# qirui-chen/RGA3-release

Measured on AMD Instinct MI355X. Metric: video-QA samples/sec (fwd+bwd) at 7B/16-frame — full RGA3 training step (Qwen2.5-VL-7B + SAM2-L + mask losses + AdamW), higher is better.
Workload: dtype bf16

## Files before the change

rga3-release_amd/csrc/attn_args.h:

```cpp
#pragma once
#include "common.h"

namespace rga3 {

struct AttnArgs {
    const unsigned short* q;
    const unsigned short* k;
    const unsigned short* v;
    unsigned short* o;
    float* lse;
    const int* cu_q;
    const int* cu_k;
    long q_st, q_sh, k_st, k_sh, v_st, v_sh, o_st, o_sh;
    int Hq, Hkv, D;
    long total_q;
    float scale_log2;
    int causal;
    float* split_o;
    float* split_lse;
    int nsplit;
    int bq_shift, bk_shift;
    const float* rope_cos;
    const float* rope_sin;
    const float* rope_kcos;
    const float* rope_ksin;
    int gx;
};

int launch_causal32(const AttnArgs& a, int nseg, int max_q, hipStream_t st);

}
```

rga3-release_amd/csrc/attn_bwd.hip:

```cpp
#include "common.h"

#include <mutex>
#include <set>

namespace rga3 {

struct AttnBwdArgs {
    const unsigned short *q, *k, *v, *o, *dout;
    unsigned short *dq, *dk, *dv;
    const float* lse;
    float* delta;
    const int *cu_q, *cu_k;
    long q_st, q_sh, k_st, k_sh, v_st, v_sh, o_st, o_sh, do_st, do_sh, dq_st, dq_sh, dk_st, dk_sh, dv_st, dv_sh;
    int Hq, Hkv, D;
    long total_q;
    float scale, scale_log2;
    int causal;
    float* dkv_ws;
    long total_k;
    int gx, gy;
};

constexpr int BT = 64;

template <int DP, int QT, int NWAVE, bool PAIR>
__global__ __launch_bounds__(64 * NWAVE) void attn_bwd_dq_kernel(AttnBwdArgs p) {
    constexpr int NT = 64 * NWAVE;
    constexpr int BLOCK_M = NWAVE * QT * 16;
    constexpr int CH = DP / 8;
    constexpr int STRIDE = DP * 2 + 32;
    constexpr int DS = DP / 32, DT = DP / 16;
    constexpr int LOADS = (BT * CH) / NT;
    static_assert((BT * CH) % NT == 0, "tile chunks must divide evenly over threads");

    extern __shared__ __attribute__((aligned(16))) char smem[];
    char* Ks = smem;
    char* Vs = smem + BT * STRIDE;

    const int tid = threadIdx.x, lane = tid & 63;
    const int wid = __builtin_amdgcn_readfirstlane(tid >> 6);
    const int g = lane >> 4, c = lane & 15;
    const Wg3 wg = xcd_decode3(p.gx, p.gy);
    const int seg = wg.z, hq = wg.y;
    const int hk = hq / (p.Hq / p.Hkv);
    const int qs = p.cu_q[seg], Lq = p.cu_q[seg + 1] - qs;
    const int ks = p.cu_k[seg], Lk = p.cu_k[seg + 1] - ks;
    const int shift = Lk - Lq;
    const int nqb = (Lq + BLOCK_M - 1) / BLOCK_M;
    int qb_first = wg.x, qb_second = -1;
    if constexpr (PAIR) {
        qb_first = nqb - 1 - wg.x;
        qb_second = wg.x;
        if (qb_second > qb_first) return;
        if (qb_second == qb_first) qb_second = -1;
    } else if (qb_first >= nqb) {
        return;
    }
    for (int pass = 0; pass < (PAIR ? 2 : 1); ++pass) {
    const int qbi = pass == 0 ? qb_first : qb_second;
    if (qbi < 0) break;
    if (pass == 1) __syncthreads();
    const int qb0 = qbi * BLOCK_M;
    const int qw0 = qb0 + wid * (QT * 16);

    bf16x8 qf[QT][DS], dof[QT][DS];
    float lse2[QT], dl[QT];
#pragma unroll
    for (int t = 0; t < QT; ++t) {
        const int qi = qw0 + t * 16 + c;
        const bool ok = qi < Lq;
#pragma unroll
        for (int ds = 0; ds < DS; ++ds) {
            const int d = ds * 32 + g * 8;
            u32x4 z = {0u, 0u, 0u, 0u}, y = {0u, 0u, 0u, 0u};
            if (ok && d < p.D) {
                z = *(const u32x4*)(p.q + (long)(qs + qi) * p.q_st + (long)hq * p.q_sh + d);
                y = *(const u32x4*)(p.dout + (long)(qs + qi) * p.do_st + (long)hq * p.do_sh + d);
            }
            qf[t][ds] = __builtin_bit_cast(bf16x8, z);
            dof[t][ds] = __builtin_bit_cast(bf16x8, y);
        }
        lse2[t] = ok ? p.lse[(long)hq * p.total_q + qs + qi] * 1.4426950408889634f : 0.f;
    }
#pragma unroll
    for (int t = 0; t < QT; ++t) {
        const int qi = qw0 + t * 16 + c;
        const bool ok = qi < Lq;
        float dp = 0.f;
#pragma unroll
        for (int ds = 0; ds < DS; ++ds) {
            const int d = ds * 32 + g * 8;
            if (ok && d < p.D) {
                const u32x4 ov = *(const u32x4*)(p.o + (long)(qs + qi) * p.o_st + (long)hq * p.o_sh + d);
                const u32x4 dv = __builtin_bit_cast(u32x4, dof[t][ds]);
#pragma unroll
                for (int i = 0; i < 4; ++i) {
                    dp += __uint_as_float(ov[i] << 16) * __uint_as_float(dv[i] << 16);
                    dp += __uint_as_float(ov[i] & 0xffff0000u) * __uint_as_float(dv[i] & 0xffff0000u);
                }
            }
        }
        dp += __shfl_xor(dp, 16, 64);
        dp += __shfl_xor(dp, 32, 64);
        dl[t] = ok ? dp : 0.f;
        if (ok && g == 0) p.delta[(long)hq * p.total_q + qs + qi] = dp;
    }

    f32x4 dqacc[QT][DT];
#pragma unroll
    for (int t = 0; t < QT; ++t)
#pragma unroll
        for (int d = 0; d < DT; ++d) dqacc[t][d] = f32x4{0.f, 0.f, 0.f, 0.f};

    int kv_end = Lk;
    if (p.causal) kv_end = min(Lk, qb0 + BLOCK_M + shift);
    if (kv_end < 0) kv_end = 0;
    const int ntiles = (kv_end + BT - 1) / BT;

    u32x4 kreg[LOADS], vreg[LOADS];
    auto load_tile = [&](int kt) {
#pragma unroll
        for (int i = 0; i < LOADS; ++i) {
            const int idx = tid + i * NT;
            const int r = idx / CH, ch = idx % CH;
            const int key = kt * BT + r;
            u32x4 zk = {0u, 0u, 0u, 0u}, zv = {0u, 0u, 0u, 0u};
            if (key < Lk && ch * 8 < p.D) {
                zk = *(const u32x4*)(p.k + (long)(ks + key) * p.k_st + (long)hk * p.k_sh + ch * 8);
                zv = *(const u32x4*)(p.v + (long)(ks + key) * p.v_st + (long)hk * p.v_sh + ch * 8);
            }
            kreg[i] = zk;
            vreg[i] = zv;
        }
    };
    auto store_tile = [&]() {
#pragma unroll
        for (int i = 0; i < LOADS; ++i) {
            const int idx = tid + i * NT;
            const int r = idx / CH, ch = idx % CH;
            *(u32x4*)(Ks + r * STRIDE + ch * 16) = kreg[i];
            *(u32x4*)(Vs + r * STRIDE + ch * 16) = vreg[i];
        }
    };

    if (ntiles > 0) load_tile(0);
    for (int kt = 0; kt < ntiles; ++kt) {
        __syncthreads();
        store_tile();
        __syncthreads();
        if (kt + 1 < ntiles) load_tile(kt + 1);
        const int k0 = kt * BT;
        const bool need_mask = (k0 + BT > Lk) || (p.causal && (k0 + BT - 1 > qb0 + shift));
#pragma unroll
        for (int t = 0; t < QT; ++t) {
            const int qi = qw0 + t * 16 + c;
            f32x4 s[4], dp[4];
#pragma unroll
            for (int j = 0; j < 4; ++j) { s[j] = f32x4{0.f, 0.f, 0.f, 0.f}; dp[j] = f32x4{0.f, 0.f, 0.f, 0.f}; }
#pragma unroll
            for (int j = 0; j < 4; ++j)
#pragma unroll
                for (int ds = 0; ds < DS; ++ds) {
                    bf16x8 kf = *(const bf16x8*)(Ks + (j * 16 + c) * STRIDE + ds * 64 + g * 16);
                    bf16x8 vf = *(const bf16x8*)(Vs + (j * 16 + c) * STRIDE + ds * 64 + g * 16);
                    s[j] = __builtin_amdgcn_mfma_f32_16x16x32_bf16(kf, qf[t][ds], s[j], 0, 0, 0);
                    dp[j] = __builtin_amdgcn_mfma_f32_16x16x32_bf16(vf, dof[t][ds], dp[j], 0, 0, 0);
                }
            bf16x8 dsf[2];
#pragma unroll
            for (int ss = 0; ss < 2; ++ss) {
                float e[8];
#pragma unroll
                for (int u = 0; u < 8; ++u) {
                    const int j = 2 * ss + (u >> 2), r = u & 3;
                    float pr = __builtin_amdgcn_exp2f(s[j][r] * p.scale_log2 - lse2[t]);
                    if (need_mask) {
                        const int key = k0 + j * 16 + 4 * g + r;
                        const bool ok = (key < Lk) && (!p.causal || key <= qi + shift);
                        pr = ok ? pr : 0.f;
                    }
                    if (qi >= Lq) pr = 0.f;
                    e[u] = pr * (dp[j][r] - dl[t]) * p.scale;
                }
                u32x4 pk;
                pk[0] = pack_bf2(e[0], e[1]); pk[1] = pack_bf2(e[2], e[3]); pk[2] = pack_bf2(e[4], e[5]); pk[3] = pack_bf2(e[6], e[7]);
                dsf[ss] = __builtin_bit_cast(bf16x8, pk);
            }
#pragma unroll
            for (int d = 0; d < DT; ++d)
#pragma unroll
                for (int ss = 0; ss < 2; ++ss) {
                    const char* a0 = Ks + (ss * 32 + 4 * g + (c >> 2)) * STRIDE + (d * 16 + 4 * (c & 3)) * 2;
                    bf16x4 lo = __builtin_amdgcn_ds_read_tr16_b64_v4bf16((__attribute__((address_space(3))) bf16x4*)(a0));
                    bf16x4 hi = __builtin_amdgcn_ds_read_tr16_b64_v4bf16((__attribute__((address_space(3))) bf16x4*)(a0 + 16 * STRIDE));
                    bf16x8 kt8;
                    kt8[0] = lo[0]; kt8[1] = lo[1]; kt8[2] = lo[2]; kt8[3] = lo[3];
                    kt8[4] = hi[0]; kt8[5] = hi[1]; kt8[6] = hi[2]; kt8[7] = hi[3];
                    dqacc[t][d] = __builtin_amdgcn_mfma_f32_16x16x32_bf16(kt8, dsf[ss], dqacc[t][d], 0, 0, 0);
                }
        }
    }
#pragma unroll
    for (int t = 0; t < QT; ++t) {
        const int qi = qw0 + t * 16 + c;
        if (qi < Lq) {
            unsigned short* row = p.dq + (long)(qs + qi) * p.dq_st + (long)hq * p.dq_sh;
#pragma unroll
            for (int d = 0; d < DT; ++d) {
                const int dd = d * 16 + 4 * g;
                if (dd < p.D) {
                    u32x2 pk;
                    pk[0] = pack_bf2(dqacc[t][d][0], dqacc[t][d][1]);
                    pk[1] = pack_bf2(dqacc[t][d][2], dqacc[t][d][3]);
                    *(u32x2*)(row + dd) = pk;
                }
            }
        }
    }
    }
}

template <int DP, int NWAVE, bool SPLIT, bool PAIR>
__global__ __launch_bounds__(64 * NWAVE) void attn_bwd_dkv_kernel(AttnBwdArgs p) {
    constexpr int NT = 64 * NWAVE;
    constexpr int BLOCK_N = NWAVE * 16;
    constexpr int CH = DP / 8;
    constexpr int STRIDE = DP * 2 + 32;
    constexpr int DS = DP / 32, DT = DP / 16;
    constexpr int LOADS = (BT * CH) / NT;
    static_assert((BT * CH) % NT == 0, "tile chunks must divide evenly over threads");

    extern __shared__ __attribute__((aligned(16))) char smem[];
    char* Qs = smem;
    char* Os = smem + BT * STRIDE;
    float* Ls = (float*)(smem + 2 * BT * STRIDE);

    const int tid = threadIdx.x, lane = tid & 63;
    const int wid = __builtin_amdgcn_readfirstlane(tid >> 6);
    const int g = lane >> 4, c = lane & 15;
    const Wg3 wg = xcd_decode3(p.gx, p.gy);
    const int seg = wg.z;
    const int group = p.Hq / p.Hkv;
    const int hk = SPLIT ? wg.y / group : wg.y;
    const int hh0 = SPLIT ? wg.y % group : 0, hh1 = SPLIT ? hh0 + 1 : group;
    const int qs = p.cu_q[seg], Lq = p.cu_q[seg + 1] - qs;
    const int ks = p.cu_k[seg], Lk = p.cu_k[seg + 1] - ks;
    const int shift = Lk - Lq;
    const int nkb = (Lk + BLOCK_N - 1) / BLOCK_N;
    int kb_first = wg.x, kb_second = -1;
    if constexpr (PAIR) {
        kb_first = wg.x;
        kb_second = nkb - 1 - wg.x;
        if (kb_first > kb_second) return;
        if (kb_second == kb_first) kb_second = -1;
    } else if (kb_first >= nkb) {
        return;
    }
    for (int pass = 0; pass < (PAIR ? 2 : 1); ++pass) {
    const int kbi = pass == 0 ? kb_first : kb_second;
    if (kbi < 0) break;
    if (pass == 1) __syncthreads();
    const int kb0 = kbi * BLOCK_N;
    const int key = kb0 + wid * 16 + c;

    bf16x8 kf[DS], vf[DS];
#pragma unroll
    for (int ds = 0; ds < DS; ++ds) {
        const int d = ds * 32 + g * 8;
        u32x4 z = {0u, 0u, 0u, 0u}, y = {0u, 0u, 0u, 0u};
        if (key < Lk && d < p.D) {
            z = *(const u32x4*)(p.k + (long)(ks + key) * p.k_st + (long)hk * p.k_sh + d);
            y = *(const u32x4*)(p.v + (long)(ks + key) * p.v_st + (long)hk * p.v_sh + d);
        }
        kf[ds] = __builtin_bit_cast(bf16x8, z);
        vf[ds] = __builtin_bit_cast(bf16x8, y);
    }
    f32x4 dkacc[DT], dvacc[DT];
#pragma unroll
    for (int d = 0; d < DT; ++d) { dkacc[d] = f32x4{0.f, 0.f, 0.f, 0.f}; dvacc[d] = f32x4{0.f, 0.f, 0.f, 0.f}; }

    int q_begin = 0;
    if (p.causal) q_begin = max(0, kb0 - shift);
    const int t0 = q_begin / BT;
    const int ntq = (Lq + BT - 1) / BT;

    u32x4 qreg[LOADS], oreg[LOADS];
    float lreg = 0.f, dreg = 0.f;
    auto load_tile = [&](int hq_, int qt_) {
#pragma unroll
        for (int i = 0; i < LOADS; ++i) {
            const int idx = tid + i * NT;
            const int r = idx / CH, ch = idx % CH;
            const int qi = qt_ * BT + r;
            u32x4 zq = {0u, 0u, 0u, 0u}, zo = {0u, 0u, 0u, 0u};
            if (qi < Lq && ch * 8 < p.D) {
                zq = *(const u32x4*)(p.q + (long)(qs + qi) * p.q_st + (long)hq_ * p.q_sh + ch * 8);
                zo = *(const u32x4*)(p.dout + (long)(qs + qi) * p.do_st + (long)hq_ * p.do_sh + ch * 8);
            }
            qreg[i] = zq;
            oreg[i] = zo;
        }
        if (tid < BT) {
            const int qi = qt_ * BT + tid;
            lreg = (qi < Lq) ? p.lse[(long)hq_ * p.total_q + qs + qi] * 1.4426950408889634f : 0.f;
            dreg = (qi < Lq) ? p.delta[(long)hq_ * p.total_q + qs + qi] : 0.f;
        }
    };
    auto store_tile = [&]() {
#pragma unroll
        for (int i = 0; i < LOADS; ++i) {
            const int idx = tid + i * NT;
            const int r = idx / CH, ch = idx % CH;
            *(u32x4*)(Qs + r * STRIDE + ch * 16) = qreg[i];
            *(u32x4*)(Os + r * STRIDE + ch * 16) = oreg[i];
        }
        if (tid < BT) {
            Ls[tid] = lreg;
            Ls[BT + tid] = dreg;
        }
    };
    if (t0 < ntq) load_tile(hk * group + hh0, t0);
    for (int hh = hh0; hh < hh1; ++hh) {
        const int hq = hk * group + hh;
        for (int qt = t0; qt < ntq; ++qt) {
            __syncthreads();
            store_tile();
            __syncthreads();
            if (qt + 1 < ntq) load_tile(hq, qt + 1);
            else if (hh + 1 < hh1) load_tile(hq + 1, t0);
            const int q0 = qt * BT;
            f32x4 s[4], dp[4];
#pragma unroll
            for (int j = 0; j < 4; ++j) { s[j] = f32x4{0.f, 0.f, 0.f, 0.f}; dp[j] = f32x4{0.f, 0.f, 0.f, 0.f}; }
#pragma unroll
            for (int j = 0; j < 4; ++j)
#pragma unroll
                for (int ds = 0; ds < DS; ++ds) {
                    bf16x8 qa = *(const bf16x8*)(Qs + (j * 16 + c) * STRIDE + ds * 64 + g * 16);
                    bf16x8 oa = *(const bf16x8*)(Os + (j * 16 + c) * STRIDE + ds * 64 + g * 16);
                    s[j] = __builtin_amdgcn_mfma_f32_16x16x32_bf16(qa, kf[ds], s[j], 0, 0, 0);
                    dp[j] = __builtin_amdgcn_mfma_f32_16x16x32_bf16(oa, vf[ds], dp[j], 0, 0, 0);
                }
            bf16x8 pf[2], dsf[2];
#pragma unroll
            for (int ss = 0; ss < 2; ++ss) {
                float e[8], f[8];
#pragma unroll
                for (int u = 0; u < 8; ++u) {
                    const int j = 2 * ss + (u >> 2), r = u & 3;
                    const int ql = j * 16 + 4 * g + r;
                    const int qi = q0 + ql;
                    float pr = __builtin_amdgcn_exp2f(s[j][r] * p.scale_log2 - Ls[ql]);
                    const bool ok = (qi < Lq) && (key < Lk) && (!p.causal || key <= qi + shift);
                    pr = ok ? pr : 0.f;
                    e[u] = pr;
                    f[u] = pr * (dp[j][r] - Ls[BT + ql]) * p.scale;
                }
                u32x4 a, b;
                a[0] = pack_bf2(e[0], e[1]); a[1] = pack_bf2(e[2], e[3]); a[2] = pack_bf2(e[4], e[5]); a[3] = pack_bf2(e[6], e[7]);
                b[0] = pack_bf2(f[0], f[1]); b[1] = pack_bf2(f[2], f[3]); b[2] = pack_bf2(f[4], f[5]); b[3] = pack_bf2(f[6], f[7]);
                pf[ss] = __builtin_bit_cast(bf16x8, a);
                dsf[ss] = __builtin_bit_cast(bf16x8, b);
            }
#pragma unroll
            for (int d = 0; d < DT; ++d)
#pragma unroll
                for (int ss = 0; ss < 2; ++ss) {
                    const int roff = (ss * 32 + 4 * g + (c >> 2)) * STRIDE + (d * 16 + 4 * (c & 3)) * 2;
                    bf16x4 ol = __builtin_amdgcn_ds_read_tr16_b64_v4bf16((__attribute__((address_space(3))) bf16x4*)(Os + roff));
                    bf16x4 oh = __builtin_amdgcn_ds_read_tr16_b64_v4bf16((__attribute__((address_space(3))) bf16x4*)(Os + roff + 16 * STRIDE));
                    bf16x4 ql_ = __builtin_amdgcn_ds_read_tr16_b64_v4bf16((__attribute__((address_space(3))) bf16x4*)(Qs + roff));
                    bf16x4 qh_ = __builtin_amdgcn_ds_read_tr16_b64_v4bf16((__attribute__((address_space(3))) bf16x4*)(Qs + roff + 16 * STRIDE));
                    bf16x8 ot, qt8;
                    ot[0] = ol[0]; ot[1] = ol[1]; ot[2] = ol[2]; ot[3] = ol[3]; ot[4] = oh[0]; ot[5] = oh[1]; ot[6] = oh[2]; ot[7] = oh[3];
                    qt8[0] = ql_[0]; qt8[1] = ql_[1]; qt8[2] = ql_[2]; qt8[3] = ql_[3]; qt8[4] = qh_[0]; qt8[5] = qh_[1]; qt8[6] = qh_[2]; qt8[7] = qh_[3];
                    dvacc[d] = __builtin_amdgcn_mfma_f32_16x16x32_bf16(ot, pf[ss], dvacc[d], 0, 0, 0);
                    dkacc[d] = __builtin_amdgcn_mfma_f32_16x16x32_bf16(qt8, dsf[ss], dkacc[d], 0, 0, 0);
                }
        }
    }
    if constexpr (SPLIT) {
        if (key < Lk) {
            const long half = (long)group * p.total_k * p.Hkv * p.D;
            float* wk = p.dkv_ws + (((long)hh0 * p.total_k + ks + key) * p.Hkv + hk) * p.D;
#pragma unroll
            for (int d = 0; d < DT; ++d) {
                const int dd = d * 16 + 4 * g;
                if (dd < p.D) {
                    *(f32x4*)(wk + dd) = dkacc[d];
                    *(f32x4*)(wk + half + dd) = dvacc[d];
                }
            }
        }
        continue;
    }
    if (key < Lk) {
        unsigned short* rk = p.dk + (long)(ks + key) * p.dk_st + (long)hk * p.dk_sh;
        unsigned short* rv = p.dv + (long)(ks + key) * p.dv_st + (long)hk * p.dv_sh;
#pragma unroll
        for (int d = 0; d < DT; ++d) {
            const int dd = d * 16 + 4 * g;
            if (dd < p.D) {
                u32x2 a, b;
                a[0] = pack_bf2(dkacc[d][0], dkacc[d][1]); a[1] = pack_bf2(dkacc[d][2], dkacc[d][3]);
                b[0] = pack_bf2(dvacc[d][0], dvacc[d][1]); b[1] = pack_bf2(dvacc[d][2], dvacc[d][3]);
                *(u32x2*)(rk + dd) = a;
                *(u32x2*)(rv + dd) = b;
            }
        }
    }
    }
}

__global__ __launch_bounds__(256) void attn_dkv_reduce_kernel(AttnBwdArgs p) {
    const int group = p.Hq / p.Hkv;
    const int d4 = p.D / 4;
    const long idx = (long)blockIdx.x * 256 + threadIdx.x;
    const long total = p.total_k * p.Hkv * d4;
    if (idx >= total) return;
    const int dd = (int)(idx % d4) * 4;
    const long row = idx / d4;
    const int hk = (int)(row % p.Hkv);
    const long key = row / p.Hkv;
    const long plane = p.total_k * p.Hkv * (long)p.D, half = (long)group * plane;
    const float* w = p.dkv_ws + row * p.D + dd;
    f32x4 sk = *(const f32x4*)w, sv = *(const f32x4*)(w + half);
    for (int h = 1; h < group; ++h) {
        sk += *(const f32x4*)(w + h * plane);
        sv += *(const f32x4*)(w + half + h * plane);
    }
    u32x2 a, b;
    a[0] = pack_bf2(sk[0], sk[1]); a[1] = pack_bf2(sk[2], sk[3]);
    b[0] = pack_bf2(sv[0], sv[1]); b[1] = pack_bf2(sv[2], sv[3]);
    *(u32x2*)(p.dk + key * p.dk_st + (long)hk * p.dk_sh + dd) = a;
    *(u32x2*)(p.dv + key * p.dv_st + (long)hk * p.dv_sh + dd) = b;
}

template <int DP>
static int launch_bwd(const AttnBwdArgs& a0, int nseg, int max_q, int max_k, hipStream_t st) {
    AttnBwdArgs a = a0;
    a.gx = 1; a.gy = 1;
    constexpr int NW = (DP == 128) ? 8 : 4;
#ifdef RGA3_BWD_DQ_QT2
    constexpr int QT = 2, NWQ = 4;
#else
    constexpr int QT = (DP >= 128) ? 1 : 2, NWQ = NW;
#endif
    constexpr int BLOCK_M = NWQ * QT * 16;
    constexpr int LDS_DQ = 2 * BT * (DP * 2 + 32);
    constexpr int LDS_DKV = 2 * BT * (DP * 2 + 32) + 2 * BT * 4;
    auto prep = [](const void* k, int lds) -> int {
        if (lds <= 48 * 1024) return 0;
        static std::mutex mu;
        static std::set<std::pair<const void*, int>> done;
        int dev = 0;
        if (hipGetDevice(&dev) != hipSuccess) dev = 0;
        std::lock_guard<std::mutex> lk(mu);
        if (done.count({k, dev})) return 0;
        hipError_t e = hipFuncSetAttribute(k, hipFuncAttributeMaxDynamicSharedMemorySize, lds);
        if (e != hipSuccess) return fail(-(int)e, "attn_bwd: hipFuncSetAttribute: %s", hipGetErrorString(e));
        done.insert({k, dev});
        return 0;
    };
    const unsigned nqb = (unsigned)cdiv(max_q, BLOCK_M), nkb = (unsigned)cdiv(max_k, 16 * NW);
    const bool pair = a.causal && nqb >= 4 && nkb >= 4;
    if (pair) {
        auto kq = attn_bwd_dq_kernel<DP, QT, NWQ, true>;
        if (int rc = prep((const void*)kq, LDS_DQ)) return rc;
        a.gx = (int)((nqb + 1) / 2); a.gy = a.Hq;
        hipLaunchKernelGGL(kq, dim3((unsigned)a.gx * (unsigned)a.gy * (unsigned)nseg), dim3(64 * NWQ), LDS_DQ, st, a);
    } else {
        auto kq = attn_bwd_dq_kernel<DP, QT, NWQ, false>;
        if (int rc = prep((const void*)kq, LDS_DQ)) return rc;
        a.gx = (int)nqb; a.gy = a.Hq;
        hipLaunchKernelGGL(kq, dim3((unsigned)a.gx * (unsigned)a.gy * (unsigned)nseg), dim3(64 * NWQ), LDS_DQ, st, a);
    }
    RGA3_CHECK_LAUNCH("attn_bwd_dq_kernel");
    const unsigned gx = pair ? (nkb + 1) / 2 : nkb;
    if (a.dkv_ws && a.Hq > a.Hkv) {
        if (pair) {
            auto ks_ = attn_bwd_dkv_kernel<DP, NW, true, true>;
            if (int rc = prep((const void*)ks_, LDS_DKV)) return rc;
            a.gx = (int)gx; a.gy = a.Hq;
            hipLaunchKernelGGL(ks_, dim3((unsigned)a.gx * (unsigned)a.gy * (unsigned)nseg), dim3(64 * NW), LDS_DKV, st, a);
        } else {
            auto ks_ = attn_bwd_dkv_kernel<DP, NW, true, false>;
            if (int rc = prep((const void*)ks_, LDS_DKV)) return rc;
            a.gx = (int)gx; a.gy = a.Hq;
            hipLaunchKernelGGL(ks_, dim3((unsigned)a.gx * (unsigned)a.gy * (unsigned)nseg), dim3(64 * NW), LDS_DKV, st, a);
        }
        RGA3_CHECK_LAUNCH("attn_bwd_dkv_kernel<split>");
        const long rows = a.total_k * a.Hkv;
        hipLaunchKernelGGL(attn_dkv_reduce_kernel, dim3((unsigned)cdiv(rows * (a.D / 4), 256)), dim3(256), 0, st, a);
        RGA3_CHECK_LAUNCH("attn_dkv_reduce_kernel");
        return 0;
    }
    if (pair) {
        auto kk = attn_bwd_dkv_kernel<DP, NW, false, true>;
        if (int rc = prep((const void*)kk, LDS_DKV)) return rc;
        a.gx = (int)gx; a.gy = a.Hkv;
        hipLaunchKernelGGL(kk, dim3((unsigned)a.gx * (unsigned)a.gy * (unsigned)nseg), dim3(64 * NW), LDS_DKV, st, a);
    } else {
        auto kk = attn_bwd_dkv_kernel<DP, NW, false, false>;
        if (int rc = prep((const void*)kk, LDS_DKV)) return rc;
        a.gx = (int)gx; a.gy = a.Hkv;
        hipLaunchKernelGGL(kk, dim3((unsigned)a.gx * (unsigned)a.gy * (unsigned)nseg), dim3(64 * NW), LDS_DKV, st, a);
    }
    RGA3_CHECK_LAUNCH("attn_bwd_dkv_kernel");
    return 0;
}

}

using namespace rga3;

extern "C" int rga3_attn_varlen_bwd(const void* q, const void* k, const void* v, const void* o, const void* dout, const float* lse,
                                    void* dq, void* dk, void* dv, float* delta_ws, const int32_t* cu_q, const int32_t* cu_k, int nseg,
                                    int max_q, int max_k, int64_t total_q, int Hq, int Hkv, int D, const int64_t* strides16, float scale,
                                    int causal, float* dkv_ws, int64_t total_k, void* stream) {
    RGA3_CHECK_ARG(q && k && v && o && dout && lse && dq && dk && dv && delta_ws && cu_q && cu_k && strides16, "attn_bwd: null pointer");
    RGA3_CHECK_ARG(nseg > 0 && max_q > 0 && max_k > 0 && total_q > 0, "attn_bwd: sizes");
    RGA3_CHECK_ARG(Hq > 0 && Hkv > 0 && Hq % Hkv == 0, "attn_bwd: Hq=%d Hkv=%d", Hq, Hkv);
    RGA3_CHECK_ARG(D >= 8 && D <= 128 && D % 8 == 0, "attn_bwd: head dim %d unsupported (multiple of 8, <= 128)", D);
    for (int i = 0; i < 16; ++i) RGA3_CHECK_ARG(strides16[i] % 4 == 0, "attn_bwd: stride %d must be a multiple of 4 elements", i);
    for (int i = 0; i < 10; ++i) RGA3_CHECK_ARG(strides16[i] % 8 == 0, "attn_bwd: input stride %d must be a multiple of 8 elements", i);
    AttnBwdArgs a;
    a.q = (const unsigned short*)q; a.k = (const unsigned short*)k; a.v = (const unsigned short*)v; a.o = (const unsigned short*)o;
    a.dout = (const unsigned short*)dout; a.dq = (unsigned short*)dq; a.dk = (unsigned short*)dk; a.dv = (unsigned short*)dv;
    a.lse = lse; a.delta = delta_ws; a.cu_q = cu_q; a.cu_k = cu_k;
    a.q_st = strides16[0]; a.q_sh = strides16[1]; a.k_st = strides16[2]; a.k_sh = strides16[3]; a.v_st = strides16[4]; a.v_sh = strides16[5];
    a.o_st = strides16[6]; a.o_sh = strides16[7]; a.do_st = strides16[8]; a.do_sh = strides16[9]; a.dq_st = strides16[10]; a.dq_sh = strides16[11];
    a.dk_st = strides16[12]; a.dk_sh = strides16[13]; a.dv_st = strides16[14]; a.dv_sh = strides16[15];
    a.Hq = Hq; a.Hkv = Hkv; a.D = D; a.total_q = total_q; a.scale = scale; a.scale_log2 = scale * 1.4426950408889634f; a.causal = causal;
    a.dkv_ws = dkv_ws; a.total_k = total_k;
    RGA3_CHECK_ARG(!dkv_ws || (total_k > 0 && D % 4 == 0), "attn_bwd: dkv_ws needs total_k");
    hipStream_t st = (hipStream_t)stream;
    if (D <= 32) return launch_bwd<32>(a, nseg, max_q, max_k, st);
    if (D <= 64) return launch_bwd<64>(a, nseg, max_q, max_k, st);
    if (D <= 96) return launch_bwd<96>(a, nseg, max_q, max_k, st);
    return launch_bwd<128>(a, nseg, max_q, max_k, st);
}
```

Measured before the change: 7.755.

## Add 32x32 MFMA causal attention backward dQ kernel for head dim 128

Adds a new dQ backward kernel for causal self-attention with head dim 128. It uses 32x32x16 bf16 MFMA, global-to-LDS async loads, transposed LDS reads and paired query blocks split across two wave groups, with the partial dQ sums combined through LDS. It fuses the delta computation into the kernel and is dispatched when shapes, strides and alignment qualify, falling back to the old kernel otherwise. The aim is higher matrix-core throughput and balanced causal work, at the cost of a large hand-scheduled kernel with a high LDS footprint.

Measured after the change: 7.769, median of 3. About the same (+0.2%).

```diff
diff --git a/rga3-release_amd/csrc/attn_args.h b/rga3-release_amd/csrc/attn_args.h
--- a/rga3-release_amd/csrc/attn_args.h
+++ b/rga3-release_amd/csrc/attn_args.h
@@ -29,4 +29,23 @@
 
 int launch_causal32(const AttnArgs& a, int nseg, int max_q, hipStream_t st);
 
+struct AttnBwdArgs {
+    const unsigned short *q, *k, *v, *o, *dout;
+    unsigned short *dq, *dk, *dv;
+    const float* lse;
+    float* delta;
+    const int *cu_q, *cu_k;
+    long q_st, q_sh, k_st, k_sh, v_st, v_sh, o_st, o_sh, do_st, do_sh, dq_st, dq_sh, dk_st, dk_sh, dv_st, dv_sh;
+    int Hq, Hkv, D;
+    long total_q;
+    float scale, scale_log2;
+    int causal;
+    float* dkv_ws;
+    long total_k;
+    int gx, gy;
+};
+
+bool bwd32_dq_ok(const AttnBwdArgs& a, int max_q, int max_k);
+int launch_bwd32_dq(const AttnBwdArgs& a, int nseg, int max_q, hipStream_t st);
+
 }
diff --git a/rga3-release_amd/csrc/attn_bwd.hip b/rga3-release_amd/csrc/attn_bwd.hip
--- a/rga3-release_amd/csrc/attn_bwd.hip
+++ b/rga3-release_amd/csrc/attn_bwd.hip
@@ -1,25 +1,9 @@
-#include "common.h"
+#include "attn_args.h"
 
 #include <mutex>
 #include <set>
 
 namespace rga3 {
-
-struct AttnBwdArgs {
-    const unsigned short *q, *k, *v, *o, *dout;
-    unsigned short *dq, *dk, *dv;
-    const float* lse;
-    float* delta;
-    const int *cu_q, *cu_k;
-    long q_st, q_sh, k_st, k_sh, v_st, v_sh, o_st, o_sh, do_st, do_sh, dq_st, dq_sh, dk_st, dk_sh, dv_st, dv_sh;
-    int Hq, Hkv, D;
-    long total_q;
-    float scale, scale_log2;
-    int causal;
-    float* dkv_ws;
-    long total_k;
-    int gx, gy;
-};
 
 constexpr int BT = 64;
 
@@ -441,11 +425,7 @@
     AttnBwdArgs a = a0;
     a.gx = 1; a.gy = 1;
     constexpr int NW = (DP == 128) ? 8 : 4;
-#ifdef RGA3_BWD_DQ_QT2
-    constexpr int QT = 2, NWQ = 4;
-#else
     constexpr int QT = (DP >= 128) ? 1 : 2, NWQ = NW;
-#endif
     constexpr int BLOCK_M = NWQ * QT * 16;
     constexpr int LDS_DQ = 2 * BT * (DP * 2 + 32);
     constexpr int LDS_DKV = 2 * BT * (DP * 2 + 32) + 2 * BT * 4;
@@ -464,7 +444,11 @@
     };
     const unsigned nqb = (unsigned)cdiv(max_q, BLOCK_M), nkb = (unsigned)cdiv(max_k, 16 * NW);
     const bool pair = a.causal && nqb >= 4 && nkb >= 4;
-    if (pair) {
+    bool dq32 = false;
+    if constexpr (DP == 128) dq32 = bwd32_dq_ok(a0, max_q, max_k);
+    if (dq32) {
+        if (int rc = launch_bwd32_dq(a0, nseg, max_q, st)) return rc;
+    } else if (pair) {
         auto kq = attn_bwd_dq_kernel<DP, QT, NWQ, true>;
         if (int rc = prep((const void*)kq, LDS_DQ)) return rc;
         a.gx = (int)((nqb + 1) / 2); a.gy = a.Hq;
@@ -475,7 +459,7 @@
         a.gx = (int)nqb; a.gy = a.Hq;
         hipLaunchKernelGGL(kq, dim3((unsigned)a.gx * (unsigned)a.gy * (unsigned)nseg), dim3(64 * NWQ), LDS_DQ, st, a);
     }
-    RGA3_CHECK_LAUNCH("attn_bwd_dq_kernel");
+    if (!dq32) RGA3_CHECK_LAUNCH("attn_bwd_dq_kernel");
     const unsigned gx = pair ? (nkb + 1) / 2 : nkb;
     if (a.dkv_ws && a.Hq > a.Hkv) {
         if (pair) {
diff --git a/rga3-release_amd/csrc/attn_bwd32.hip b/rga3-release_amd/csrc/attn_bwd32.hip
--- /dev/null
+++ b/rga3-release_amd/csrc/attn_bwd32.hip
@@ -0,0 +1,326 @@
+#include "attn_args.h"
+#include <type_traits>
+
+#ifndef RGA3_BWD32_DQ
+#define RGA3_BWD32_DQ 1
+#endif
+
+namespace rga3 {
+
+namespace {
+constexpr int B32_KT = 64;
+constexpr int B32_QB = 128;
+constexpr int B32_ROWB = 256;
+constexpr int B32_HALF = B32_KT * B32_ROWB;
+constexpr int B32_LDS = 8 * B32_HALF;
+constexpr int B32_MIN_Q = 4 * B32_QB;
+
+__device__ __forceinline__ int b32_swz(int row) { return ((row & 3) << 2) | ((row >> 2) & 3); }
+}
+
+__global__ __launch_bounds__(512) void attn_bwd32_dq_kernel(AttnBwdArgs p) {
+    extern __shared__ __attribute__((aligned(16))) char smem[];
+    const int tid = threadIdx.x, lane = tid & 63;
+    const int wid = __builtin_amdgcn_readfirstlane(tid >> 6);
+    const int grp = wid >> 2, w4 = wid & 3;
+    const int r = lane & 31, h = lane >> 5;
+
+    const unsigned lid = xcd_remap(blockIdx.x, gridDim.x);
+    const int hq = (int)(lid % (unsigned)p.Hq);
+    const int bx = (int)((lid / (unsigned)p.Hq) % (unsigned)p.gx);
+    const int seg = (int)(lid / ((unsigned)p.Hq * (unsigned)p.gx));
+    const int hk = hq / (p.Hq / p.Hkv);
+    const int qs = p.cu_q[seg], Lq = p.cu_q[seg + 1] - qs;
+    const int ks = p.cu_k[seg], Lk = p.cu_k[seg + 1] - ks;
+    const int shift = Lk - Lq;
+    const int nqb = (Lq + B32_QB - 1) / B32_QB;
+    const int qbH = nqb - 1 - bx;
+    if (bx > qbH) return;
+    const int qbL = (bx == qbH) ? -1 : bx;
+    auto ktiles = [&](int qb) {
+        const int e = min(Lk, qb * B32_QB + B32_QB + shift);
+        return e > 0 ? (e + B32_KT - 1) / B32_KT : 0;
+    };
+    const int kH = ktiles(qbH), kL = qbL >= 0 ? min(ktiles(qbL), kH) : 0;
+    const int c = (kH + kL + 1) >> 1;
+
+    const unsigned short* kbase = p.k + (long)ks * p.k_st + (long)hk * p.k_sh;
+    const unsigned short* vbase = p.v + (long)ks * p.v_st + (long)hk * p.v_sh;
+
+    char* const KX = smem;
+    char* const VX = smem + 2 * B32_HALF;
+    char* const KY = smem + 4 * B32_HALF;
+    char* const VY = smem + 6 * B32_HALF;
+
+    auto run = [&](auto GRP) {
+    constexpr int G = decltype(GRP)::value;
+    int lane_ = tid & 63;
+    asm volatile("" : "+v"(lane_));
+    const int lane = lane_, r = lane & 31, h = lane >> 5;
+    unsigned dko[2], dvo[2];
+#pragma unroll
+    for (int j = 0; j < 2; ++j) {
+        const int blk = 2 * wid + j;
+        const int row = 4 * blk + (lane >> 4);
+        const int lc = (lane & 15) ^ (((lane >> 4) << 2) | (blk & 3));
+        dko[j] = (unsigned)(row * (int)p.k_st + lc * 8);
+        dvo[j] = (unsigned)(row * (int)p.v_st + lc * 8);
+    }
+    auto issue_img = [&](const unsigned short* base, long st, const unsigned (&d)[2], int tile, char* img) {
+        if (tile * B32_KT + B32_KT <= Lk) {
+            const unsigned short* tb = base + (long)tile * B32_KT * st;
+#pragma unroll
+            for (int j = 0; j < 2; ++j) {
+                unsigned o_ = d[j];
+                asm volatile("" : "+v"(o_));
+                __builtin_amdgcn_global_load_lds((gbl_void*)(tb + o_), (lds_void*)(img + (2 * wid + j) * 1024), 16, 0, 0);
+            }
+        } else {
+#pragma unroll
+            for (int j = 0; j < 2; ++j) {
+                const int blk = 2 * wid + j;
+                const int row = 4 * blk + (lane >> 4);
+                const int lc = (lane & 15) ^ (((lane >> 4) << 2) | (blk & 3));
+                const int key = min(tile * B32_KT + row, Lk - 1);
+                __builtin_amdgcn_global_load_lds((gbl_void*)(base + (long)key * st + lc * 8), (lds_void*)(img + blk * 1024), 16, 0, 0);
+            }
+        }
+    };
+    auto issue_slot = [&](int j) {
+        if (j >= c) return;
+        const int b = (j & 1) * B32_HALF;
+        issue_img(kbase, p.k_st, dko, j, KX + b);
+        issue_img(vbase, p.v_st, dvo, j, VX + b);
+        const int ty = c + j - kL;
+        if (j >= kL && ty < kH) {
+            issue_img(kbase, p.k_st, dko, ty, KY + b);
+            issue_img(vbase, p.v_st, dvo, ty, VY + b);
+        }
+    };
+
+    const int koff0 = r * B32_ROWB + ((h ^ b32_swz(r)) << 4);
+    auto koff = [&](int kk) { return koff0 ^ (kk << 5); };
+    int tro0[2];
+    {
+        const int g1 = (lane >> 4) & 1, q_ = (lane >> 2) & 3, p_ = lane & 3;
+#pragma unroll
+        for (int jj = 0; jj < 2; ++jj) {
+            const int x = (q_ << 2) | ((2 * jj + h) & 3);
+            const int lc = 2 * g1 + (p_ >> 1);
+            tro0[jj] = (8 * jj + 4 * h + q_) * B32_ROWB + ((lc ^ x) << 4) + 8 * (p_ & 1);
+        }
+    }
+    auto tro = [&](int jj, int b) { return tro0[jj] ^ (b << 6); };
+
+    bf16x8 qf[8], dof[8];
+    f32x16 dqa[4];
+    float lse2, dl;
+    int qw0;
+    const float cs = p.scale_log2;
+    auto start_rows = [&](int qb, bool write_delta) {
+        int r_ = r, h_ = h;
+        asm volatile("" : "+s"(qb), "+v"(r_), "+v"(h_));
+        const int r = r_, h = h_;
+        qw0 = qb * B32_QB + w4 * 32;
+        const int qi = min(qw0 + r, Lq - 1);
+        const unsigned short* qrow = p.q + (long)(qs + qi) * p.q_st + (long)hq * p.q_sh + 8 * h;
+        const unsigned short* drow = p.dout + (long)(qs + qi) * p.do_st + (long)hq * p.do_sh + 8 * h;
+        const unsigned short* orow = p.o + (long)(qs + qi) * p.o_st + (long)hq * p.o_sh + 8 * h;
+#pragma unroll
+        for (int kk = 0; kk < 8; ++kk) {
+            qf[kk] = *(const bf16x8*)(qrow + 16 * kk);
+            dof[kk] = *(const bf16x8*)(drow + 16 * kk);
+        }
+        float dp = 0.f;
+#pragma unroll
+        for (int kk = 0; kk < 8; ++kk) {
+            const u32x4 ov = *(const u32x4*)(orow + 16 * kk);
+            const u32x4 dv = __builtin_bit_cast(u32x4, dof[kk]);
+#pragma unroll
+            for (int i = 0; i < 4; ++i) {
+                dp += __uint_as_float(ov[i] << 16) * __uint_as_float(dv[i] << 16);
+                dp += __uint_as_float(ov[i] & 0xffff0000u) * __uint_as_float(dv[i] & 0xffff0000u);
+            }
+        }
+        dp += __shfl_xor(dp, 32, 64);
+        dl = dp;
+        lse2 = p.lse[(long)hq * p.total_q + qs + qi] * 1.4426950408889634f;
+        if (write_delta && h == 0 && qw0 + r < Lq) p.delta[(long)hq * p.total_q + qs + qi] = dp;
+#pragma unroll
+        for (int b = 0; b < 4; ++b)
+#pragma unroll
+            for (int i = 0; i < 16; ++i) dqa[b][i] = 0.f;
+#pragma unroll
+        for (int kk = 0; kk < 8; ++kk) {
+            asm volatile("" : "+v"(qf[kk]));
+            asm volatile("" : "+v"(dof[kk]));
+        }
+    };
+    auto store_rows = [&]() {
+        int qw = qw0, r_ = r, h_ = h;
+        asm volatile("" : "+s"(qw), "+v"(r_), "+v"(h_));
+        const int r = r_, h = h_;
+        const int qi = qw + r;
+        unsigned short* orow = p.dq + (long)(qs + min(qi, Lq - 1)) * p.dq_st + (long)hq * p.dq_sh + 8 * h;
+#pragma unroll
+        for (int b = 0; b < 4; ++b)
+#pragma unroll
+            for (int i4 = 0; i4 < 4; i4 += 2) {
+                unsigned ax = pack_bf2(dqa[b][4 * i4], dqa[b][4 * i4 + 1]), ay = pack_bf2(dqa[b][4 * i4 + 2], dqa[b][4 * i4 + 3]);
+                unsigned bx_ = pack_bf2(dqa[b][4 * i4 + 4], dqa[b][4 * i4 + 5]), by = pack_bf2(dqa[b][4 * i4 + 6], dqa[b][4 * i4 + 7]);
+                const auto r0 = __builtin_amdgcn_permlane32_swap(ax, bx_, false, false);
+                const auto r1 = __builtin_amdgcn_permlane32_swap(ay, by, false, false);
+                if (qi < Lq) *(u32x4*)(orow + 32 * b + 8 * i4) = u32x4{(unsigned)r0[0], (unsigned)r1[0], (unsigned)r0[1], (unsigned)r1[1]};
+            }
+    };
+
+    bool onH = (G == 0) || (qbL < 0);
+    auto slot_tile = [&](int j) { return (G == 0 || j < kL) ? j : c + j - kL; };
+    auto slot_live = [&](int j, bool on_h) {
+        const int t = (G == 0 || j < kL) ? j : c + j - kL;
+        return j < c && t < (on_h ? kH : kL) && qw0 < Lq && t * B32_KT <= qw0 + 31 + shift;
+    };
+
+    auto tile = [&](int j) {
+        const bool x = (G == 0 || j < kL);
+        const char* Kb = (x ? KX : KY) + (j & 1) * B32_HALF;
+        const char* Vb = (x ? VX : VY) + (j & 1) * B32_HALF;
+        const int k0 = slot_tile(j) * B32_KT;
+        const bool need_mask = (k0 + B32_KT > Lk) || (k0 + B32_KT - 1 > qw0 + shift);
+        const int lim = min(Lk - 1, qw0 + r + shift);
+#pragma unroll
+        for (int kb = 0; kb < 2; ++kb) {
+            f32x16 s, dp;
+#pragma unroll
+            for (int i = 0; i < 16; ++i) { s[i] = 0.f; dp[i] = 0.f; }
+            const char* Kr = Kb + kb * 32 * B32_ROWB;
+            const char* Vr = Vb + kb * 32 * B32_ROWB;
+            bf16x8 kf[2], vf[2];
+            kf[0] = *(const bf16x8*)(Kr + koff(0));
+            vf[0] = *(const bf16x8*)(Vr + koff(0));
+#pragma unroll
+            for (int kk = 0; kk < 8; ++kk) {
+                if (kk + 1 < 8) {
+                    kf[(kk + 1) & 1] = *(const bf16x8*)(Kr + koff(kk + 1));
+                    vf[(kk + 1) & 1] = *(const bf16x8*)(Vr + koff(kk + 1));
+                }
+                s = __builtin_amdgcn_mfma_f32_32x32x16_bf16(kf[kk & 1], qf[kk], s, 0, 0, 0);
+                dp = __builtin_amdgcn_mfma_f32_32x32x16_bf16(vf[kk & 1], dof[kk], dp, 0, 0, 0);
+            }
+            __builtin_amdgcn_sched_group_barrier(0x100, 2, 0);
+#pragma unroll
+            for (int kk = 0; kk < 7; ++kk) {
+                __builtin_amdgcn_sched_group_barrier(0x100, 2, 0);
+                __builtin_amdgcn_sched_group_barrier(0x008, 2, 0);
+            }
+            __builtin_amdgcn_sched_group_barrier(0x008, 2, 0);
+#pragma unroll
+            for (int i = 0; i < 16; ++i) {
+                float pr = __builtin_amdgcn_exp2f(__builtin_fmaf(s[i], cs, -lse2));
+                if (need_mask) {
+                    const int key = k0 + kb * 32 + (i & 3) + 8 * (i >> 2) + 4 * h;
+                    pr = (key > lim) ? 0.f : pr;
+                }
+                s[i] = pr * (dp[i] - dl) * p.scale;
+            }
+            bf16x8 pb[2];
+#pragma unroll
+            for (int ss = 0; ss < 2; ++ss) {
+                u32x4 pk;
+                pk[0] = pack_bf2(s[8 * ss + 0], s[8 * ss + 1]);
+                pk[1] = pack_bf2(s[8 * ss + 2], s[8 * ss + 3]);
+                pk[2] = pack_bf2(s[8 * ss + 4], s[8 * ss + 5]);
+                pk[3] = pack_bf2(s[8 * ss + 6], s[8 * ss + 7]);
+                pb[ss] = __builtin_bit_cast(bf16x8, pk);
+            }
+#pragma unroll
+            for (int ss = 0; ss < 2; ++ss)
+#pragma unroll
+                for (int b = 0; b < 4; ++b) {
+                    const char* a0 = Kr + 16 * ss * B32_ROWB;
+                    const bf16x4 lo = __builtin_amdgcn_ds_read_tr16_b64_v4bf16((__attribute__((address_space(3))) bf16x4*)(a0 + tro(0, b)));
+                    const bf16x4 hi = __builtin_amdgcn_ds_read_tr16_b64_v4bf16((__attribute__((address_space(3))) bf16x4*)(a0 + tro(1, b)));
+                    bf16x8 kt;
+                    kt[0] = lo[0]; kt[1] = lo[1]; kt[2] = lo[2]; kt[3] = lo[3];
+                    kt[4] = hi[0]; kt[5] = hi[1]; kt[6] = hi[2]; kt[7] = hi[3];
+                    dqa[b] = __builtin_amdgcn_mfma_f32_32x32x16_bf16(kt, pb[ss], dqa[b], 0, 0, 0);
+                }
+        }
+    };
+
+    issue_slot(0);
+    start_rows(onH ? qbH : qbL, G == 0 || !onH);
+    asm volatile("s_waitcnt vmcnt(0)" ::: "memory");
+    __builtin_amdgcn_s_barrier();
+    bool live = slot_live(0, onH);
+    for (int it = 0; it < c; ++it) {
+        issue_slot(it + 1);
+        if (live) tile(it);
+        if constexpr (G == 1) {
+            if (!onH && it + 1 >= kL) {
+                store_rows();
+                start_rows(qbH, false);
+                onH = true;
+            }
+        }
+        live = slot_live(it + 1, onH);
+        asm volatile("s_waitcnt vmcnt(0)" ::: "memory");
+        __builtin_amdgcn_s_barrier();
+    }
+
+    if (G == 1 && !onH) {
+        store_rows();
+        start_rows(qbH, false);
+    }
+    float* const mo = (float*)smem;
+    if constexpr (G == 1) {
+#pragma unroll
+        for (int b = 0; b < 4; ++b)
+#pragma unroll
+            for (int i4 = 0; i4 < 4; ++i4)
+                *(f32x4*)(mo + (((w4 * 16 + b * 4 + i4) * 64 + lane) << 2)) = f32x4{dqa[b][4 * i4], dqa[b][4 * i4 + 1], dqa[b][4 * i4 + 2], dqa[b][4 * i4 + 3]};
+    }
+    __syncthreads();
+    if constexpr (G == 0) {
+#pragma unroll
+        for (int b = 0; b < 4; ++b)
+#pragma unroll
+            for (int i4 = 0; i4 < 4; ++i4) {
+                const f32x4 ob = *(const f32x4*)(mo + (((w4 * 16 + b * 4 + i4) * 64 + lane) << 2));
+#pragma unroll
+                for (int e = 0; e < 4; ++e) dqa[b][4 * i4 + e] += ob[e];
+            }
+        store_rows();
+    }
+    };
+    if (grp == 0) run(std::integral_constant<int, 0>{});
+    else run(std::integral_constant<int, 1>{});
+}
+
+bool bwd32_dq_ok(const AttnBwdArgs& a, int max_q, int max_k) {
+#if RGA3_BWD32_DQ
+    if (a.D != 128 || !a.causal || a.cu_q != a.cu_k || max_q != max_k || max_q < B32_MIN_Q) return false;
+    const long st[16] = {a.q_st, a.q_sh, a.k_st, a.k_sh, a.v_st, a.v_sh, a.o_st, a.o_sh, a.do_st, a.do_sh, a.dq_st, a.dq_sh, a.dk_st, a.dk_sh, a.dv_st, a.dv_sh};
+    for (long s : st)
+        if (s % 8 != 0) return false;
+    const uintptr_t ptrs = (uintptr_t)a.q | (uintptr_t)a.k | (uintptr_t)a.v | (uintptr_t)a.o | (uintptr_t)a.dout | (uintptr_t)a.dq | (uintptr_t)a.dk | (uintptr_t)a.dv;
+    if (ptrs & 15) return false;
+    return a.k_st > 0 && a.v_st > 0 && a.k_st < (1 << 24) && a.v_st < (1 << 24);
+#else
+    (void)a; (void)max_q; (void)max_k;
+    return false;
+#endif
+}
+
+int launch_bwd32_dq(const AttnBwdArgs& a, int nseg, int max_q, hipStream_t st) {
+    static LdsGrant lds_grant;
+    if (int rc = grant_dyn_lds((const void*)attn_bwd32_dq_kernel, B32_LDS, lds_grant, "attn_bwd32_dq")) return rc;
+    AttnBwdArgs b = a;
+    const unsigned nqb = (unsigned)cdiv(max_q, B32_QB);
+    b.gx = (int)((nqb + 1) / 2); b.gy = a.Hq;
+    hipLaunchKernelGGL(attn_bwd32_dq_kernel, dim3((unsigned)b.gx * (unsigned)a.Hq * (unsigned)nseg), dim3(512), B32_LDS, st, b);
+    RGA3_CHECK_LAUNCH("attn_bwd32_dq_kernel");
+    return 0;
+}
+
+}
```
